# moritzmeister/hops-examples

Hardware: AMD Instinct MI355X
Metric: images/sec MNIST CNN + steps/sec Chicago-taxi DNN at 1/2/4/8 MI355X (higher is better)
Workload: dtype bf16; 1 GPU; model=MNIST CNN (experiment.mirrored model, 1394282 params), Adadelta(1.0), global_batch=32, per_gpu_batch=32, parallelism=dp1, engine=PersistentMnistStep, hipgraph=False, steps_per_execution=32, warmup_steps_run=5

## Files before the change

csrc/ops/bindings.cpp:

```cpp
#include <pybind11/pybind11.h>
#include <pybind11/stl.h>

#include <algorithm>
#include <stdexcept>
#include <string>
#include <tuple>
#include <utility>
#include <vector>

#if defined(HOPSX_DEBUG) && HOPSX_DEBUG
#define HOPSX_DEBUG_BUILD 1
#else
#define HOPSX_DEBUG_BUILD 0
#endif

#include "ops_api.h"
extern "C" int hopsx_mnist_persist_occupancy(int dp);
extern "C" void hopsx_mnist_persist_reload_knobs();
extern "C" int hopsx_pad_cin(const float* w, long R, int C, int cp, float* out, void* out16, hipStream_t st);
extern "C" int hopsx_unpad_cin_add(float* gpad, long R, int C, int cp, float* tgt, hipStream_t st);

namespace py = pybind11;
extern "C" void hopsx_mlp_head_debug(void* p);
extern "C" int hopsx_conv2d_bwd_pair_opt(const void* dy, const void* w, const int* geom, void* dx, const void* yprev,
// ... 168 lines not shown
    }
    persist_slots[slot] = PersistSlot{std::move(p), std::move(iv), std::move(fv)};
    return slot;
  });
  m.def("mnist_persist_slot", [](int slot, u st) {
    if (slot < 0 || slot >= (int)persist_slots.size()) return (int)hipErrorInvalidValue;
    const PersistSlot& a = persist_slots[slot];
    return hopsx_mnist_persist(a.p.data(), (int)a.p.size(), a.iv.data(), (int)a.iv.size(), a.fv.data(),
                               (int)a.fv.size(), S(st));
  });
  m.def("mnist_eval", [](std::vector<uint64_t> p, std::vector<long> iv, std::vector<float> fv, u st) {
    return hopsx_mnist_eval(p.data(), (int)p.size(), iv.data(), (int)iv.size(), fv.data(), (int)fv.size(), S(st));
  });
  m.def("mnist_eval_tile", []() { return hopsx_mnist_eval_tile(); });
  m.def("mnist_persist_reload_knobs", []() { hopsx_mnist_persist_reload_knobs(); });
  m.def("mnist_persist_occupancy", [](int dp) { return hopsx_mnist_persist_occupancy(dp); });
  m.def("pad_cin", [](u w, long R, int C, int cp, u out, u out16, u st) {
    return hopsx_pad_cin(P<float>(w), R, C, cp, P<float>(out), P<void>(out16), S(st));
  });
  m.def("unpad_cin_add", [](u g, long R, int C, int cp, u tgt, u st) {
    return hopsx_unpad_cin_add(P<float>(g), R, C, cp, P<float>(tgt), S(st));
  });
  m.def("mnist_persist_geom", []() {
    std::vector<long> g(23);
    hopsx_mnist_persist_geom(g.data());
    return g;
  });
  m.def("widedeep_step", [](std::vector<uint64_t> p, std::vector<long> iv, std::vector<float> fv, u st) {
    return hopsx_widedeep_step(p.data(), (int)p.size(), iv.data(), (int)iv.size(), fv.data(), (int)fv.size(),
                               S(st));
  });
  m.def("conv2d_fwd_pool_ok", [](std::vector<int> g, int act, int pk) { return hopsx_conv_fwd_pool_ok(g.data(), act, pk); });
  m.def("conv2d_fwd_pool", [](u x, u w, std::vector<int> g, u out, u am, u bias, int act, float p, u rng,
                              unsigned salt, int pk, u st) {
    return hopsx_conv2d_fwd_pool(P<void>(x), P<void>(w), g.data(), P<void>(out), P<void>(am), P<float>(bias), act, p,
                                 P<unsigned long long>(rng), salt, pk, S(st));
  });
  m.def("conv2d_fwd_pool_in_ok", [](std::vector<int> g0, std::vector<int> g, int act) {
    return hopsx_conv_fwd_pool_in_ok(g0.data(), g.data(), act);
  });
  m.def("conv2d_fwd_pool_in", [](u x0, float xscale, float xshift, u w0, u b0, int act0, std::vector<int> g0, u y1,
                                 u w, std::vector<int> g, u out, u am, u bias, int act, float p, u rng, unsigned salt,
                                 u st) {
    return hopsx_conv2d_fwd_pool_in(P<void>(x0), xscale, xshift, P<void>(w0), P<float>(b0), act0, g0.data(),
                                    P<void>(y1), P<void>(w), g.data(), P<void>(out), P<void>(am), P<float>(bias), act,
                                    p, P<unsigned long long>(rng), salt, S(st));
  });
// ... 227 lines not shown
```

csrc/ops/mnist_persist.hip:

```cpp
#include "common.h"
#include "optim_core.h"

namespace mnistp {

constexpr int B = 32;
constexpr int C1 = 32, C2 = 64, HID = 128, NCLS = 10;
constexpr int PH = 13, NPOS = PH * PH;
constexpr int KIN = NPOS * C2;
constexpr int NCONV = C2 * 128 + C2 + C1 * 4 + C1;
constexpr int OFF_B2 = C2 * 128, OFF_W1 = OFF_B2 + C2, OFF_B1 = OFF_W1 + C1 * 4;
constexpr int SLICE = 52, NSLICE = (NCONV + SLICE - 1) / SLICE;
constexpr int NRED = 19;
constexpr int NHEAD = B;
constexpr int GRID = NPOS + NHEAD;
constexpr int PAY = 272;
constexpr int PAY_DH = 0, PAY_H = 128, PAY_DL = 256, PAY_LOSS = 268, PAY_COR = 269;
constexpr int FL_A = 0, FL_B = 256, FL_C = 512, FL_D = 768, FL_WORDS = 1024;
constexpr int FL_EPOCH = FL_WORDS - 2;
constexpr int D_F32 = OFF_B2 * 2;
constexpr int D_BYTES = D_F32 + (NCONV - OFF_B2) * 4;
constexpr int TGB_N = NHEAD * (HID / 2);
constexpr int TG_WORDS = 2 * 2 * TGB_N;
static_assert(FL_WORDS % 2 == 0 && TGB_N % 256 == 0, "granules are 8-B aligned; every thread owns TGB_N / 256");

constexpr int W1S = 72, W2S = 136, C1S = 40, PLS = 72, DHS = 136, DCS = 136;

constexpr int L_W1 = 0;
constexpr int L_W2 = L_W1 + HID * W1S * 2;
constexpr int L_CW1 = L_W2 + C2 * W2S * 2;
constexpr int L_CB1 = L_CW1 + C1 * 4 * 4;
constexpr int L_CB2 = L_CB1 + C1 * 4;
constexpr int L_XIN = L_CB2 + C2 * 4;
constexpr int L_C1 = L_XIN + B * 16 * 4;
constexpr int L_POOL = L_C1 + B * 9 * C1S * 2;
constexpr int L_AM = L_POOL + B * PLS * 2;
constexpr int L_DH = L_AM + B * C2;
constexpr int L_DC2 = L_DH + B * DHS * 2;
constexpr int L_STG = L_DC2 + C2 * DCS * 2;
constexpr int L_RED = L_STG + NCONV * 4;
constexpr int L_SL = L_RED + 1024 * 4;
constexpr int L_KEEP = L_SL + 3 * 64 * 4;
constexpr int LDS_BYTES = L_KEEP + B * C2;

constexpr int H_W2 = 0;
constexpr int H_B2 = H_W2 + 3 * NCLS * HID * 4;
constexpr int H_B1 = H_B2 + 3 * 16 * 4;
// ... 230 lines not shown
__device__ __forceinline__ unsigned ecode(int phase, int s) {
  return 0x80000000u | ((unsigned)phase << 24) | (((unsigned)s & 0xFFFu) << 12) | (blockIdx.x & 0xFFFu);
}

__device__ __forceinline__ bf16_raw f2bf(float f) { return __builtin_bit_cast(bf16_raw, (__bf16)f); }

__device__ __forceinline__ bf16x8 lds8(const bf16_raw* p) { return *(const bf16x8*)p; }
__device__ __forceinline__ bf16x8 lds_tr(const bf16_raw* p1, const bf16_raw* p2) {
  const bf16x4 v1 = __builtin_amdgcn_ds_read_tr16_b64_v4i16((lds_v4_ptr)(p1));
  const bf16x4 v2 = __builtin_amdgcn_ds_read_tr16_b64_v4i16((lds_v4_ptr)(p2));
  return (bf16x8){v1[0], v1[1], v1[2], v1[3], v2[0], v2[1], v2[2], v2[3]};
}
__device__ __forceinline__ f32x4 mfma(bf16x8 a, bf16x8 b, f32x4 c) {
  return __builtin_amdgcn_mfma_f32_16x16x32_bf16(a, b, c, 0, 0, 0);
}

__device__ __forceinline__ long conv_idx(const Args& a, int j) {
  if (j < OFF_B2) return a.off[2] + j;
  if (j < OFF_W1) return a.off[3] + (j - OFF_B2);
  if (j < OFF_B1) return a.off[0] + (j - OFF_W1);
  return a.off[1] + (j - OFF_B1);
}

__device__ __forceinline__ void stamp(const Args& a, int s, int ph) {
  if (a.dbg && threadIdx.x == 0) a.dbg[((long)blockIdx.x * a.nsteps + s) * 16 + ph] = (unsigned long long)wall_clock64();
}

__device__ __forceinline__ void granule_store(unsigned long long* g, unsigned epoch, unsigned value) {
  __hip_atomic_store((gu64*)g, ((unsigned long long)epoch << 32) | value, __ATOMIC_RELAXED, __HIP_MEMORY_SCOPE_AGENT);
}
__device__ __forceinline__ unsigned long long granule_load(const unsigned long long* g) {
  return __hip_atomic_load((gu64*)g, __ATOMIC_RELAXED, __HIP_MEMORY_SCOPE_AGENT);
}
__device__ __forceinline__ bool gate_tags(const unsigned long long* g, int gi, unsigned epoch, int need, unsigned* err,
                                       unsigned code, int* s_ok, long long tmo) {
  if (threadIdx.x < 64) {
    const int lane = threadIdx.x;
    const bool mine = lane < NHEAD;
    int good = 1;
    const long long t0 = wall_clock64();
    for (unsigned spins = 0;; ++spins) {
      const unsigned e = flag_load(err);
      const unsigned long long x = mine ? granule_load(g + lane * (HID / 2) + gi) : 0ull;
      const bool hit = mine && (unsigned)(x >> 32) == epoch;
      if (__popcll(__ballot(hit)) >= need) break;
      if (__builtin_amdgcn_readfirstlane(e) != 0u) {
        good = 0;
        break;
      }
      if ((spins & 15u) == 15u && wall_clock64() - t0 > tmo) {
        if (lane == 0) atomicCAS(err, 0u, code);
        good = 0;
        break;
      }
      __builtin_amdgcn_s_sleep(1);
    }
    if (lane == 0) *s_ok = good;
  }
  __syncthreads();
  const int v = *s_ok;
  return v != 0;
}
template <int N, class F>
__device__ __forceinline__ bool sweep_tags(const unsigned long long* g, int tid, unsigned epoch, unsigned* err,
                                        unsigned code, int* s_fail, long long tmo, F put) {
  unsigned pend = (1u << N) - 1u;
  unsigned long long x[N];
#pragma unroll
  for (int k = 0; k < N; ++k) x[k] = granule_load(g + tid + 256 * k);
  unsigned e = flag_load(err);
  const long long t0 = wall_clock64();
  for (unsigned spins = 0;; ++spins) {
#pragma unroll
    for (int k = 0; k < N; ++k)
      if (((pend >> k) & 1u) && (unsigned)(x[k] >> 32) == epoch) {
        put(tid + 256 * k, (unsigned)x[k]);
        pend &= ~(1u << k);
      }
    if (!__any(pend != 0u)) break;
    bool bad = __builtin_amdgcn_readfirstlane(e) != 0u;
    if (!bad && (spins & 15u) == 15u && wall_clock64() - t0 > tmo) {
      if ((threadIdx.x & 63) == 0) atomicCAS(err, 0u, code);
      bad = true;
    }
    if (bad) {
      if ((threadIdx.x & 63) == 0) *s_fail = 1;
      break;
    }
#pragma unroll
    for (int k = 0; k < N; ++k)
      if ((pend >> k) & 1u) x[k] = granule_load(g + tid + 256 * k);
    e = flag_load(err);
// ... 41 lines not shown
        g2[ii][j][r] = a.s2[ai];
        W1[n * W1S + co] = f2bf(wm[ii][j][r]);
      }
  auto put_conv = [&](int j, float v) {
    if (j < OFF_B2) W2[(j >> 7) * W2S + (j & 127)] = f2bf(v);
    else if (j < OFF_W1) CB2[j - OFF_B2] = v;
    else if (j < OFF_B1) CW1[j - OFF_W1] = v;
    else CB1[j - OFF_B1] = v;
  };
  {
    constexpr int NJ = (NCONV + 255) / 256;
    float cv[NJ];
#pragma unroll
    for (int q = 0; q < NJ; ++q) {
      const int j = tid + 256 * q;
      cv[q] = j < NCONV ? a.master[conv_idx(a, j)] : 0.f;
    }
#pragma unroll
    for (int q = 0; q < NJ; ++q) {
      const int j = tid + 256 * q;
      if (j < NCONV) put_conv(j, cv[q]);
    }
  }
  const bool owner = p < NSLICE;
  if (owner && tid < SLICE) {
    const int e = p * SLICE + tid;
    if (e < NCONV) {
      const long ci = conv_idx(a, e);
      SLm[tid] = a.master[ci];
      SL1[tid] = a.s1[ci];
      SL2[tid] = a.s2[ci];
    }
  }
  const int xb = tid >> 3, xr = (tid >> 1) & 3, xh = tid & 1;
  auto xload = [&](int s) -> unsigned {
    const long bt = (long)((cur0 + s) % a.nbatch);
    const unsigned char* q = a.xs + (bt * B + xb) * 784 + (2 * ph + xr) * 28 + 2 * pw + 2 * xh;
    return *(const unsigned short*)q;
  };
  unsigned xv = xload(0);
  const float P = a.drop_p, inv = P > 0.f ? 1.f / (1.f - P) : 1.f;
  unsigned char* KEEP = smem + L_KEEP;
  auto draw_keep = [&](int s) {
    const unsigned long long ctr = ctr0 + (unsigned long long)s;
    const uint64_t dkey = (uint64_t)seed ^ ((uint64_t)a.salt * 0xD1B54A32D192ED03ull) ^
                          ((uint64_t)ctr * 0x8CB92BA72F3D8DD7ull);
    for (int e = threadIdx.x; e < B * C2; e += 256) {
      const int b = e >> 6, co = e & 63;
      const long gb = (long)a.rank * B + b;
      KEEP[e] = P > 0.f ? (unsigned char)(uniform01(dkey, (uint64_t)((gb * NPOS + p) * C2 + co)) >= P) : 1;
    }
  };
  draw_keep(0);
  __syncthreads();

  for (int s = 0; s < a.nsteps; ++s) {
    const unsigned ep = (unsigned)(eb + (unsigned long long)s + 1ull);
    const int par = s & 1;
    int oz;
    asm volatile("v_mov_b32 %0, 0" : "=v"(oz));
    const int tid = threadIdx.x + oz, lane = tid & 63, w = tid >> 6, fr = lane & 15, fq = lane >> 4;
    const int tq = fr >> 2, tp = fr & 3, xb = tid >> 3, xr = (tid >> 1) & 3, xh = tid & 1;
    stamp(a, s, 0);
    XIN[xb * 16 + xr * 4 + 2 * xh] = (float)(xv & 0xFFu) * a.xscale + a.xshift;
    XIN[xb * 16 + xr * 4 + 2 * xh + 1] = (float)(xv >> 8) * a.xscale + a.xshift;
    __syncthreads();
    {
      const int ci = tid & 31, bg = tid >> 5;
      const float k0 = CW1[ci * 4 + 0], k1 = CW1[ci * 4 + 1], k2 = CW1[ci * 4 + 2], k3 = CW1[ci * 4 + 3];
      const float bias = CB1[ci];
#pragma unroll
      for (int u = 0; u < 4; ++u) {
        const int b = bg * 4 + u;
        const float* xi = XIN + b * 16;
#pragma unroll
        for (int py = 0; py < 3; ++py)
#pragma unroll
          for (int px = 0; px < 3; ++px) {
            float v = bias;
            v = fmaf(xi[py * 4 + px], k0, v);
            v = fmaf(xi[py * 4 + px + 1], k1, v);
            v = fmaf(xi[(py + 1) * 4 + px], k2, v);
            v = fmaf(xi[(py + 1) * 4 + px + 1], k3, v);
            C1[(b * 9 + py * 3 + px) * C1S + ci] = f2bf(fmaxf(v, 0.f));
          }
      }
    }
    __syncthreads();
    {
      f32x4 acc[2][4];
#pragma unroll
      for (int ii = 0; ii < 2; ++ii)
#pragma unroll
        for (int j = 0; j < 4; ++j) acc[ii][j] = (f32x4){0.f, 0.f, 0.f, 0.f};
#pragma unroll
      for (int kk = 0; kk < 4; ++kk) {
        const int di = kk >> 1, dj = kk & 1;
        bf16x8 af[2];
#pragma unroll
        for (int ii = 0; ii < 2; ++ii) {
          const int b = 4 * (2 * w + ii) + (fr >> 2), q = fr & 3;
          const int pos = ((q >> 1) + di) * 3 + (q & 1) + dj;
          af[ii] = lds8(C1 + (b * 9 + pos) * C1S + fq * 8);
        }
#pragma unroll
        for (int j = 0; j < 4; ++j) {
          const bf16x8 bfr = lds8(W2 + (j * 16 + fr) * W2S + kk * 32 + fq * 8);
#pragma unroll
          for (int ii = 0; ii < 2; ++ii) acc[ii][j] = mfma(af[ii], bfr, acc[ii][j]);
        }
      }
// ... 53 lines not shown
    }
    __syncthreads();
    {
      const auto R = rsrc(a.slabA + ((long)par * NPOS + p) * (B * HID));
#pragma unroll
      for (int k = 0; k < 4; ++k) {
        const int idx = tid + 256 * k;
        st_sc1(R, idx * 16, *(const f32x4*)(STG + idx * 4));
      }
      drain();
      __syncthreads();
      if (tid == 0) flag_store(a.flags + FL_A + p, ep);
    }
    const unsigned gep = (unsigned)(xs0 + s + 1);
    if constexpr (DP) {
      const int c0 = w * 16 + 4 * tp;
      const f32x4 f = __builtin_bit_cast(f32x4, lds_tr(POOL + (8 * fq + tq) * PLS + c0, POOL + (8 * fq + tq + 4) * PLS + c0));
      for (int r = 0; r < a.world; ++r) {
        if (r == a.rank) continue;
        st_sys(rsrc(a.xbuf[r] + XO_POOL + (par * XMAX + xslot(a, r)) * XS_POOL + (long)p * 4096), (w * 64 + lane) * 16, f);
      }
    }
    if (s + 1 < a.nsteps) xv = xload(s + 1);
    stamp(a, s, 2);
    if (a.hand & 1) {
      const unsigned long long* TB = (const unsigned long long*)(a.flags + FL_WORDS) + par * TGB_N;
      const unsigned code = s ? ecode(2, s) : ecode(12, 0);
      const long long tmo = s ? a.tmo : a.tmo0;
      if (!gate_tags(TB, p & (HID / 2 - 1), ep, (a.hand >> 8), a.err, code, s_ok, tmo)) return;
      if (!sweep_tags<TGB_N / 256>(TB, tid, ep, a.err, code, s_ok + 2, tmo, [&](int idx, unsigned v) {
            *(unsigned*)(DH + (idx >> 6) * DHS + 2 * (idx & 63)) = v;
          }))
        return;
      if constexpr (DP) {
        drain();
        __syncthreads();
        if (tid < 64) raise_peers(a, XF_POOL + p, NPOS, gep);
      }
      stamp(a, s, 3);
    } else {
    if (!wait_all(a.flags + FL_B, NHEAD, ep, a.err, s ? ecode(2, s) : ecode(12, 0), a.acquire, s_ok,
                  s ? a.tmo : a.tmo0, a.pollw_b, a.stagger, (a.hand & 2)))
      return;
    if constexpr (DP) {
      drain();
      __syncthreads();
      if (tid < 64) raise_peers(a, XF_POOL + p, NPOS, gep);
    }
    stamp(a, s, 3);
    {
      const auto R = rsrc(a.slabB + (long)par * NHEAD * PAY);
#pragma unroll
      for (int k = 0; k < 4; ++k) {
        const int idx = tid + 256 * k, b = idx >> 5, n4 = idx & 31;
        const f32x4 v = ld_sc1(R, (b * PAY + PAY_DH + n4 * 4) * 4);
        *(bf16x4*)(DH + b * DHS + n4 * 4) =
            (bf16x4){(short)f2bf(v[0]), (short)f2bf(v[1]), (short)f2bf(v[2]), (short)f2bf(v[3])};
      }
    }
    __syncthreads();
    }
    f32x4 gw[2][4], dp[2];
    {
      if constexpr (!DP) {
#pragma unroll
      for (int ii = 0; ii < 2; ++ii) {
        const int n0 = (2 * w + ii) * 16 + 4 * tp;
        const bf16x8 af = lds_tr(DH + (8 * fq + tq) * DHS + n0, DH + (8 * fq + tq + 4) * DHS + n0);
#pragma unroll
        for (int j = 0; j < 4; ++j) {
          const int c0 = j * 16 + 4 * tp;
          const bf16x8 bfr = lds_tr(POOL + (8 * fq + tq) * PLS + c0, POOL + (8 * fq + tq + 4) * PLS + c0);
          gw[ii][j] = mfma(af, bfr, (f32x4){0.f, 0.f, 0.f, 0.f});
        }
      }
      }
      dp[0] = dp[1] = (f32x4){0.f, 0.f, 0.f, 0.f};
#pragma unroll
      for (int kk = 0; kk < 4; ++kk) {
        const int k1 = kk * 32 + 8 * fq + tq;
        const bf16x8 bfr = lds_tr(W1 + k1 * W1S + w * 16 + 4 * tp, W1 + (k1 + 4) * W1S + w * 16 + 4 * tp);
#pragma unroll
        for (int i = 0; i < 2; ++i) dp[i] = mfma(lds8(DH + (i * 16 + fr) * DHS + kk * 32 + fq * 8), bfr, dp[i]);
      }
    }
// ... 87 lines not shown
#pragma unroll
        for (int py = 0; py < 3; ++py)
#pragma unroll
          for (int px = 0; px < 3; ++px) {
            const int pos = py * 3 + px;
            const float dd = (short)C1[(b * 9 + pos) * C1S + ci] > 0 ? d[pos] : 0.f;
            gk[0] = fmaf(dd, xi[py * 4 + px], gk[0]);
            gk[1] = fmaf(dd, xi[py * 4 + px + 1], gk[1]);
            gk[2] = fmaf(dd, xi[(py + 1) * 4 + px], gk[2]);
            gk[3] = fmaf(dd, xi[(py + 1) * 4 + px + 1], gk[3]);
            gk[4] += dd;
          }
      }
#pragma unroll
      for (int k = 0; k < 5; ++k) {
        gk[k] += __shfl_xor(gk[k], 16, 64);
        gk[k] += __shfl_xor(gk[k], 32, 64);
      }
      if (fq == 0) {
#pragma unroll
        for (int k = 0; k < 5; ++k) RED[(mh * 32 + ci) * 5 + k] = gk[k];
      }
    }
    __syncthreads();
    if (tid < 32 * 5) {
      const int ci = tid / 5, k = tid - ci * 5;
      const float v = RED[ci * 5 + k] + RED[(32 + ci) * 5 + k];
      if (k < 4) STG[OFF_W1 + ci * 4 + k] = v;
      else STG[OFF_B1 + ci] = v;
    }
    __syncthreads();
    stamp(a, s, 5);
    {
      const auto R = rsrc(a.slabC + ((long)par * NPOS + p) * NCONV);
      const int idx = OFF_B2 / 4 + tid;
      if (idx < NCONV / 4) st_sc1(R, idx * 16, *(const f32x4*)(STG + idx * 4));
      drain();
      __syncthreads();
      if (tid == 0) flag_store(a.flags + FL_C + p, ep);
    }
    stamp(a, s, 6);
    if (owner) {
      if (!wait_all(a.flags + FL_C, NPOS, ep, a.err, ecode(3, s), a.acquire, s_ok, a.tmo, a.pollw_c, a.stagger, (a.hand & 2)))
        return;
      stamp(a, s, 7);
      const int e0 = p * SLICE;
      if (tid < 13 * NRED) {
        const int j = tid % 13, g = tid / 13;
        f32x4 acc = (f32x4){0.f, 0.f, 0.f, 0.f};
        if (e0 + 4 * j < NCONV) {
          const auto R = rsrc(a.slabC + (long)par * NPOS * NCONV);
          constexpr int NK = (NPOS + NRED - 1) / NRED;
          f32x4 v[NK];
#pragma unroll
          for (int k = 0; k < NK; ++k) {
            const int pp = g + NRED * k;
            v[k] = pp < NPOS ? ld_sc1(R, (pp * NCONV + e0 + 4 * j) * 4) : (f32x4){0.f, 0.f, 0.f, 0.f};
          }
#pragma unroll
          for (int k = 0; k < NK; ++k) acc += v[k];
        }
        *(f32x4*)(RED + g * SLICE + 4 * j) = acc;
      }
      __syncthreads();
      const int e = e0 + tid;
// ... 75 lines not shown
#pragma unroll
          for (int ii = 0; ii < 2; ++ii)
            af[b][ii] = __builtin_bit_cast(bf16x8, ld_sys(XD, (int)(r * XS_DHT) + ((2 * w + ii) * 64 + lane) * 16));
#pragma unroll
          for (int j = 0; j < 4; ++j)
            bfr[b][j] = __builtin_bit_cast(bf16x8, ld_sys(XP, (int)(r * XS_POOL) + (j * 64 + lane) * 16));
        }
      };
#pragma unroll
      for (int r = 0; r < PF - 1; ++r)
        if (r < a.world) fetch(r, r);
#pragma unroll
      for (int r = 0; r < XMAX; ++r) {
        if (r < a.world) {
          if (r + PF - 1 < XMAX && r + PF - 1 < a.world) fetch(r + PF - 1, (r + PF - 1) % PF);
#pragma unroll
          for (int ii = 0; ii < 2; ++ii)
#pragma unroll
            for (int j = 0; j < 4; ++j)
              gw[ii][j] += mfma(af[r % PF][ii], bfr[r % PF][j], (f32x4){0.f, 0.f, 0.f, 0.f});
        }
      }
    }
#pragma unroll
    for (int ii = 0; ii < 2; ++ii)
#pragma unroll
      for (int j = 0; j < 4; ++j)
#pragma unroll
        for (int r = 0; r < 4; ++r) {
          wm[ii][j][r] = adadelta(wm[ii][j][r], gw[ii][j][r] * hp.gscale, g1[ii][j][r], g2[ii][j][r], hp);
          W1[((2 * w + ii) * 16 + fq * 4 + r) * W1S + j * 16 + fr] = f2bf(wm[ii][j][r]);
        }
    if (s + 1 < a.nsteps) draw_keep(s + 1);
    stamp(a, s, 9);
    if (!wait_all(a.flags + FL_D, NSLICE, ep, a.err, ecode(4, s), a.acquire, s_ok, a.tmo, a.pollw_d, a.stagger,
                  (a.hand & 2)))
      return;
    stamp(a, s, 10);
    {
      const auto R = rsrc((const unsigned char*)a.slabD + (long)par * D_BYTES);
      constexpr int NB = OFF_B2 * 2 / 16;
      constexpr int NF = (NCONV - OFF_B2) / 4;
      f32x4 dv[NB / 256 + 1];
#pragma unroll
      for (int k = 0; k < NB / 256; ++k) dv[k] = ld_sc1(R, (tid + 256 * k) * 16);
      dv[NB / 256] = tid < NF ? ld_sc1(R, D_F32 + tid * 16) : (f32x4){0.f, 0.f, 0.f, 0.f};
#pragma unroll
      for (int k = 0; k < NB / 256; ++k) {
        const int c = tid + 256 * k;
        *(f32x4*)(W2 + (c >> 4) * W2S + (c & 15) * 8) = dv[k];
      }
      if (tid < NF) {
        const int j = OFF_B2 + tid * 4;
        float* dst = j < OFF_W1 ? CB2 + (j - OFF_B2) : (j < OFF_B1 ? CW1 + (j - OFF_W1) : CB1 + (j - OFF_B1));
        *(f32x4*)dst = dv[NB / 256];
      }
    }
    __syncthreads();
    stamp(a, s, 11);
  }

#pragma unroll
  for (int ii = 0; ii < 2; ++ii)
#pragma unroll
    for (int j = 0; j < 4; ++j)
#pragma unroll
      for (int r = 0; r < 4; ++r) {
        const int n = (2 * w + ii) * 16 + fq * 4 + r, co = j * 16 + fr;
        const long ai = a.off[4] + (long)n * KIN + p * C2 + co;
        a.master[ai] = wm[ii][j][r];
        a.s1[ai] = g1[ii][j][r];
        a.s2[ai] = g2[ii][j][r];
        a.shadow[ai] = f2bf(wm[ii][j][r]);
      }
  if (owner && tid < SLICE) {
    const int e = p * SLICE + tid;
    if (e < NCONV) {
      const long ci = conv_idx(a, e);
      a.master[ci] = SLm[tid];
      a.s1[ci] = SL1[tid];
      a.s2[ci] = SL2[tid];
      a.shadow[ci] = f2bf(SLm[tid]);
    }
  }
  stamp(a, a.nsteps - 1, 14);
  if (p == 0 && tid == 0) {
    if constexpr (DP) a.xstep[0] = xs0 + a.nsteps;
    a.cursor[0] = (cur0 + a.nsteps) % a.nbatch;
    *(unsigned long long*)(a.flags + FL_EPOCH) = eb + (unsigned long long)a.nsteps;
    a.rng[1] = ctr0 + (unsigned long long)a.nsteps;
    if (a.step_dev) a.step_dev[0] += (float)a.nsteps;
  }
}

template <bool DP>
__device__ __forceinline__ void head_wg(const Args& a, unsigned char* smem, int* s_ok, const OptHP& hp,
                                        long long cur0, long long xs0, unsigned long long eb) {
  const int i = blockIdx.x - NPOS;
  const int tid = threadIdx.x, lane = tid & 63;
  float* HW = (float*)(smem + H_W2);
  float* HW1 = HW + NCLS * HID;
  float* HW2 = HW1 + NCLS * HID;
  float* HB2 = (float*)(smem + H_B2);
  float* HB1 = (float*)(smem + H_B1);
  float* RED = (float*)(smem + H_RED);
  float* HH = (float*)(smem + H_H);
// ... 348 lines not shown
  a.rng = (unsigned long long*)p[7];
  a.step_dev = (float*)p[8];
  a.hp_dev = (const float*)p[9];
  a.slabA = (float*)p[10];
  a.slabB = (float*)p[11];
  a.slabC = (float*)p[12];
  a.slabD = (float*)p[13];
  a.flags = (unsigned*)p[14];
  a.err = (unsigned*)p[15];
  a.out = (float*)p[16];
  a.dbg = (unsigned long long*)p[17];
  for (int k = 0; k < 8; ++k) a.off[k] = iv[k];
  a.nbatch = iv[8];
  a.salt = (unsigned)iv[9];
  a.nsteps = (int)iv[10];
  a.acquire = (int)iv[12];
  a.world = world;
  a.rank = rank;
  a.loopback = (int)iv[15];
  a.xfence = (int)iv[17];
  a.tmo = (long long)iv[16] * 100000ll;
  a.tmo0 = a.tmo;
  static int kn_ok = 0, kn_pollw, kn_stagger, kn_a, kn_b, kn_c, kn_d, kn_head1w, kn_memset, kn_coop;
  static int kn_tagged, kn_gate, kn_poll1;
  static long kn_start_ms;
  if (!kn_ok || g_persist_reload) {
    auto pw = [&](const char* name, long dflt) {
      const long v = hopsx_env_int(name, dflt);
      return (int)(v >= 1 && v <= 4 ? v : 1);
    };
    kn_pollw = pw("HOPSX_PERSIST_POLLW", 1);
    kn_stagger = (int)hopsx_env_int("HOPSX_PERSIST_STAGGER", 12);
    kn_a = pw("HOPSX_PERSIST_POLLW_A", kn_pollw);
    kn_b = pw("HOPSX_PERSIST_POLLW_B", kn_pollw);
    kn_c = pw("HOPSX_PERSIST_POLLW_C", 4);
    kn_d = pw("HOPSX_PERSIST_POLLW_D", kn_pollw);
    kn_head1w = (int)hopsx_env_int("HOPSX_PERSIST_HEAD1W", 1);
    kn_memset = (int)hopsx_env_int("HOPSX_PERSIST_MEMSET", 0);
    kn_coop = (int)hopsx_env_int("HOPSX_PERSIST_COOP", 0);
    kn_start_ms = hopsx_env_int("HOPSX_PERSIST_START_MS", 50);
    kn_tagged = hopsx_env_int("HOPSX_PERSIST_TAGGED", 1) != 0;
    const long gt = hopsx_env_int("HOPSX_PERSIST_GATE", NHEAD / 2);
    kn_gate = (int)(gt >= 1 && gt <= NHEAD ? gt : NHEAD / 2);
    kn_poll1 = hopsx_env_int("HOPSX_PERSIST_POLL1", 1) != 0;
    kn_ok = 1;
    g_persist_reload = 0;
  }
  a.pollw = kn_pollw;
  a.stagger = kn_stagger;
  a.pollw_a = kn_a;
  a.pollw_b = kn_b;
  a.pollw_c = kn_c;
  a.pollw_d = kn_d;
  a.head1w = kn_head1w;
  a.hand = kn_tagged | (kn_poll1 << 1) | (kn_gate << 8);
  if (kn_start_ms > 0 && kn_start_ms * 100000ll < a.tmo) a.tmo0 = kn_start_ms * 100000ll;
  a.inv_gb = 1.f / (float)(world * B);
  if (dp) {
    a.xstep = (long long*)p[18];
    for (int r = 0; r < world; ++r) {
      a.xbuf[r] = (unsigned char*)p[19 + r];
      a.xflag[r] = (unsigned*)p[19 + world + r];
      if (!a.xbuf[r] || !a.xflag[r] || ((uint64_t)a.xbuf[r] & 15)) return (int)hipErrorInvalidValue;
    }
  }
  a.drop_p = fv[0];
  a.xscale = fv[1];
  a.xshift = fv[2];
  a.hp = OptHP{fv[3], fv[4], fv[5], fv[6], fv[7], 0.f, 0.f, 0.f};
  static bool attr[2] = {false, false};
  const void* fn = dp ? (const void*)mnist_persist_k<true> : (const void*)mnist_persist_k<false>;
  if (!attr[dp]) {
    const hipError_t e = hipFuncSetAttribute(fn, hipFuncAttributeMaxDynamicSharedMemorySize, LDS_BYTES);
    if (e != hipSuccess) return (int)e;
    attr[dp] = true;
  }
  if (kn_memset) {
    const hipError_t e = hipMemsetAsync(a.flags, 0, FL_WORDS * sizeof(unsigned), st);
// ... 29 lines not shown
  g[0] = B;
  g[1] = NPOS;
  g[2] = NHEAD;
  g[3] = GRID;
  g[4] = NCONV;
  g[5] = NSLICE;
  g[6] = SLICE;
  g[7] = PAY;
  g[8] = FL_WORDS;
  g[9] = LDS_BYTES;
  g[10] = D_BYTES;
  g[11] = X_BYTES;
  g[12] = XF_WORDS;
  g[13] = XMAX;
  g[14] = XO_POOL;
  g[15] = XS_POOL;
  g[16] = XO_DHT;
  g[17] = XS_DHT;
  g[18] = XO_FC2;
  g[19] = XS_FC2;
  g[20] = XO_CONV;
  g[21] = XS_CONV;
  g[22] = TG_WORDS;
}
```

hops_examples_amd/runtime/persist.py:

```python
from __future__ import annotations

import os

import torch

_GEOM = None


def _ext():
    from ..ops import _C

    return _C.ext()


def geometry() -> dict:
    global _GEOM
    if _GEOM is None:
        g = _ext().mnist_persist_geom()
        _GEOM = dict(zip(["batch", "npos", "nhead", "grid", "nconv", "nslice", "slice", "pay", "flag_words",
                          "lds_bytes", "d_bytes", "x_bytes", "xflag_words", "max_ranks", "xo_pool", "xs_pool",
                          "xo_dht", "xs_dht", "xo_fc2", "xs_fc2", "xo_conv", "xs_conv", "tag_words"], g))
    return _GEOM


class PersistentError(RuntimeError):
    pass


def flagship_layers(model):
    from .. import nn as hnn
    from ..models.mnist import MirroredMnistCNN

    names = ("conv1", "conv2", "pool", "fc1", "fc2")
    L = [getattr(model, n, None) for n in names]
    if any(x is None for x in L):
        return None
    c1, c2, pool, f1, f2 = L

    def conv_ok(c, cin, cout):
        return (isinstance(c, hnn.Conv2d) and c.in_channels == cin and c.out_channels == cout
                and tuple(c.kernel_size) == (2, 2) and c.activation == "relu" and c.bias is not None
                and c.cfg.get("stride", 1) in (1, (1, 1)) and c.cfg.get("padding", 0) in (0, "valid", (0, 0))
                and c.cfg.get("dilation", 1) in (1, (1, 1)))

    def dense_ok(d, fin, fout, act):
# ... 7 lines not shown
    return L if ok and type(model).forward is MirroredMnistCNN.forward else None


def _device_cus(dev) -> int:
    return int(torch.cuda.get_device_properties(dev).multi_processor_count)


def _occupancy(dp: bool) -> int:
    return int(_ext().mnist_persist_occupancy(int(dp)))


def launchable(dev, world: int = 1) -> tuple[bool, str]:
    g = geometry()
    cus = _device_cus(dev)
    if cus < g["grid"]:
        return False, f"{cus} CUs < the persistent grid of {g['grid']} workgroups"
    occ = _occupancy(world > 1)
    if occ < 1:
        return False, f"occupancy {occ} workgroups per CU"
    return True, "ok"


class PersistentMnistStep:
    PARAMS = ("conv1.weight", "conv1.bias", "conv2.weight", "conv2.bias", "fc1.weight", "fc1.bias",
              "fc2.weight", "fc2.bias")

    @staticmethod
    def supported(model, opt, batch: int, world: int = 1) -> bool:
        from ..optim import Adadelta

        if os.environ.get("HOPSX_PERSIST", "1") != "1":
            return False
        if world > 1 and (os.environ.get("HOPSX_PERSIST_DP", "1") != "1" or world > geometry()["max_ranks"]):
            return False
        a = getattr(opt, "arena", None)
        if not (isinstance(opt, Adadelta) and batch == 32 and a is not None and a.device.type == "cuda"
                and a.shadow is not None and opt._sl.start == 0 and opt._sl.stop >= a.numel and model.training
                and flagship_layers(model) is not None):
            return False
        return launchable(a.device, world)[0]

    def __init__(self, model, opt, steps_per_launch: int = 32, debug_stamps: bool = False, world: int | None = None,
                 loopback: int = 0, timeout_s: float | None = None, exchange=None):
        from ..ops.functional import rng_state
        from ..parallel import dist as hdist

        a = opt.arena
        self.model, self.opt, self.arena = model, opt, a
        dev = a.device
        self.device = dev
        g = geometry()
        self.geom = g
        named = dict(model.named_parameters())
        self.offs = [int(named[n]._hx_off) for n in self.PARAMS]
        self.s1 = a.state("adadelta_s0")
        self.s2 = a.state("adadelta_s1")
        self.spl = max(1, int(os.environ.get("HOPSX_PERSIST_STEPS", steps_per_launch)))
        f32 = dict(device=dev, dtype=torch.float32)
        B, npos, nh = g["batch"], g["npos"], g["nhead"]
        self.slabA = torch.empty(2 * npos * B * 128, **f32)
        self.slabB = torch.empty(2 * nh * g["pay"], **f32)
        self.slabC = torch.empty(2 * npos * g["nconv"], **f32)
        self.slabD = torch.empty(2 * g["d_bytes"] // 4, **f32)
        self._flagbuf = torch.zeros(g["flag_words"] + g["tag_words"], device=dev, dtype=torch.int32)
        self.flags = self._flagbuf[:g["flag_words"]]
        self.tags = self._flagbuf[g["flag_words"]:]
        self.err = torch.zeros(4, device=dev, dtype=torch.int32)
        self.out = torch.zeros(2 * self.spl, **f32)
        self.cursor = torch.zeros(1, device=dev, dtype=torch.int64)
        self.rng = rng_state(dev)
        self.dbg = torch.zeros(g["grid"] * self.spl * 16, device=dev, dtype=torch.int64) if debug_stamps else None
        self.acquire = int(os.environ.get("HOPSX_PERSIST_ACQUIRE", "0"))
        self.loopback = int(loopback)
        self.xfence = int(os.environ.get("HOPSX_PERSIST_XFENCE", "0"))
        if exchange is not None:
            self.world, self.rank = int(exchange.world), 0
        elif self.loopback > 1:
            self.world, self.rank = self.loopback, 0
        else:
            self.world = int(world) if world is not None else hdist.world_size()
            self.rank = hdist.rank() if self.world > 1 else 0
        if self.world > g["max_ranks"]:
            raise ValueError(f"the persistent step supports <= {g['max_ranks']} ranks")
        default_t = "60" if self.world > 1 else "2"
        self.timeout_ms = int(1000 * float(timeout_s or os.environ.get("HOPSX_PERSIST_TIMEOUT_S", default_t)))
        self._xptrs: list[int] = []
        self._owned: list[int] = []
        self._opened: list[int] = []
        self.exchange = exchange
        self.selftest_report: dict | None = None
        if exchange is not None:
            self.xstep = torch.zeros(1, device=self.device, dtype=torch.int64)
            exchange.attach(self)
        elif self.world > 1:
# ... 304 lines not shown
    def eager(self, x, y):
        return self(x, y)

    def prepare_resident(self, xs, ys, n=None) -> None:
        nb = self._check_data(xs, ys)
        if n:
            self.opt.sync_hp()
            hp = [float(v) for v in self.opt._hp()]
            for k in {min(int(n), self.spl), int(n) % self.spl} - {0}:
                self._arg_slot(self._launch_key(xs, ys, nb, k, hp), xs, ys, nb, k, hp)

    def losses(self, k: int) -> torch.Tensor:
        return self.out[: 2 * k].view(k, 2)

    def check(self) -> None:
        e = int(self.err[0].item()) & 0xFFFFFFFF
        if e:
            self._flagbuf.zero_()
            phase, step, wg = (e >> 24) & 0x7F, (e >> 12) & 0xFFF, e & 0xFFF
            if phase == 12:
                raise PersistentError(f"mnist_persist: the grid's workgroups were not co-resident (workgroup {wg} "
                                      "waited out step 0's local hand-off: another kernel holds CUs this launch "
                                      "needs); arena state of the failed launch is partial")
            raise PersistentError(f"mnist_persist: hand-off wait timed out (phase {phase}, step {step}, "
                                  f"workgroup {wg}); arena state of the failed launch is partial")

    def phase_stamps(self, k: int) -> torch.Tensor:
        if self.dbg is None:
            raise RuntimeError("construct with debug_stamps=True")
        return self.dbg.view(self.geom["grid"], self.spl, 16)[:, :k]


_M32 = 0xFFFFFFFF


def _mix32(x: torch.Tensor) -> torch.Tensor:
    x = x ^ (x >> 16)
    x = (x * 0x7FEB352D) & _M32
    x = x ^ (x >> 15)
    x = (x * 0x846CA68B) & _M32
    return x ^ (x >> 16)


def dropout_keep(seed: int, ctr: int, salt: int, idx: torch.Tensor, p: float) -> torch.Tensor:
    m64 = (1 << 64) - 1
    key = (seed ^ ((salt * 0xD1B54A32D192ED03) & m64) ^ ((ctr * 0x8CB92BA72F3D8DD7) & m64)) & m64
    ka, kb = key & _M32, key >> 32
    h = _mix32((_mix32((idx & _M32) ^ ka) + kb) & _M32)
    return (h & 0xFFFFFF).to(torch.float64) * (1.0 / 16777216.0) >= p


class _RoundFwd(torch.autograd.Function):

# ... 94 lines not shown
```

Before: 1.361 million images/sec.

## Split conv gradient hand-off so small conv params reduce via tags and overlap conv1

Adds a split mode, on by default, to the persistent MNIST step. The small conv parameters (conv2 bias, conv1 weight and bias) get their gradients reduced through per-position tagged granules and a few dedicated owners. Only the conv2 weight goes through the sliced slab C/D path, and the next step's input and conv1 forward is computed while waiting for the conv2 weight broadcast. The dropout mask draw and the fc1 Adadelta update are also moved earlier to overlap with the hand-off waits. In exchange, the flag buffer and the control flow grow, and there are new tag regions and extra wait phases that could add polling cost.

```diff
diff --git a/csrc/ops/bindings.cpp b/csrc/ops/bindings.cpp
--- a/csrc/ops/bindings.cpp
+++ b/csrc/ops/bindings.cpp
@@ -214,7 +214,7 @@
     return hopsx_unpad_cin_add(P<float>(g), R, C, cp, P<float>(tgt), S(st));
   });
   m.def("mnist_persist_geom", []() {
-    std::vector<long> g(23);
+    std::vector<long> g(30);
     hopsx_mnist_persist_geom(g.data());
     return g;
   });
diff --git a/csrc/ops/mnist_persist.hip b/csrc/ops/mnist_persist.hip
--- a/csrc/ops/mnist_persist.hip
+++ b/csrc/ops/mnist_persist.hip
@@ -22,6 +22,18 @@
 constexpr int TGB_N = NHEAD * (HID / 2);
 constexpr int TG_WORDS = 2 * 2 * TGB_N;
 static_assert(FL_WORDS % 2 == 0 && TGB_N % 256 == 0, "granules are 8-B aligned; every thread owns TGB_N / 256");
+constexpr int NSMALL = NCONV - OFF_B2;
+constexpr int NSL2 = (OFF_B2 + SLICE - 1) / SLICE;
+constexpr int NSOWN = NSMALL / 2;
+constexpr int FL_C1 = FL_WORDS + TG_WORDS, FC1_WORDS = 256;
+constexpr int TGC_N = NSMALL * NPOS;
+constexpr int TGC_OFF = FL_C1 + FC1_WORDS, TGC_WORDS = 2 * 2 * TGC_N;
+constexpr int TGD_OFF = TGC_OFF + TGC_WORDS, TGD_WORDS = 2 * 2 * NSMALL;
+constexpr int SP_WORDS = FC1_WORDS + TGC_WORDS + TGD_WORDS;
+constexpr int NSTAMP = 20;
+static_assert(NSMALL % 2 == 0 && NSOWN <= NSL2 && NSL2 <= NSLICE && 2 * NPOS <= 512 && NSMALL <= 256 &&
+                  TGC_OFF % 2 == 0 && TGD_OFF % 2 == 0 && SLICE + 2 <= 64 && SLICE % 2 == 0,
+              "split geometry: 8-B aligned granules, two sweep passes per small owner, state rows of 64");
 
 constexpr int W1S = 72, W2S = 136, C1S = 40, PLS = 72, DHS = 136, DCS = 136;
 
@@ -298,8 +310,8 @@
   return a.off[1] + (j - OFF_B1);
 }
 
-__device__ __forceinline__ void stamp(const Args& a, int s, int ph) {
-  if (a.dbg && threadIdx.x == 0) a.dbg[((long)blockIdx.x * a.nsteps + s) * 16 + ph] = (unsigned long long)wall_clock64();
+__device__ __forceinline__ void stamp(const Args& a, int s, int ph, int t = 0) {
+  if (a.dbg && threadIdx.x == t) a.dbg[((long)blockIdx.x * a.nsteps + s) * NSTAMP + ph] = (unsigned long long)wall_clock64();
 }
 
 __device__ __forceinline__ void granule_store(unsigned long long* g, unsigned epoch, unsigned value) {
@@ -339,11 +351,14 @@
 }
 template <int N, class F>
 __device__ __forceinline__ bool sweep_tags(const unsigned long long* g, int tid, unsigned epoch, unsigned* err,
-                                        unsigned code, int* s_fail, long long tmo, F put) {
-  unsigned pend = (1u << N) - 1u;
+                                        unsigned code, int* s_fail, long long tmo, F put, int n = 256 * N) {
+  unsigned pend = 0u;
   unsigned long long x[N];
 #pragma unroll
-  for (int k = 0; k < N; ++k) x[k] = granule_load(g + tid + 256 * k);
+  for (int k = 0; k < N; ++k) {
+    if (tid + 256 * k < n) pend |= 1u << k;
+    x[k] = tid + 256 * k < n ? granule_load(g + tid + 256 * k) : 0ull;
+  }
   unsigned e = flag_load(err);
   const long long t0 = wall_clock64();
   for (unsigned spins = 0;; ++spins) {
@@ -431,15 +446,21 @@
       if (j < NCONV) put_conv(j, cv[q]);
     }
   }
-  const bool owner = p < NSLICE;
-  if (owner && tid < SLICE) {
+  const bool split = DP ? false : (a.hand & 4) != 0;
+  if (p < (split ? NSL2 : NSLICE) && tid < SLICE) {
     const int e = p * SLICE + tid;
-    if (e < NCONV) {
+    if (e < (split ? OFF_B2 : NCONV)) {
       const long ci = conv_idx(a, e);
       SLm[tid] = a.master[ci];
       SL1[tid] = a.s1[ci];
       SL2[tid] = a.s2[ci];
     }
+  }
+  if (split && p < NSOWN && tid < 2) {
+    const long ci = conv_idx(a, OFF_B2 + 2 * p + tid);
+    SLm[SLICE + tid] = a.master[ci];
+    SL1[SLICE + tid] = a.s1[ci];
+    SL2[SLICE + tid] = a.s2[ci];
   }
   const int xb = tid >> 3, xr = (tid >> 1) & 3, xh = tid & 1;
   auto xload = [&](int s) -> unsigned {
@@ -471,6 +492,7 @@
     const int tid = threadIdx.x + oz, lane = tid & 63, w = tid >> 6, fr = lane & 15, fq = lane >> 4;
     const int tq = fr >> 2, tp = fr & 3, xb = tid >> 3, xr = (tid >> 1) & 3, xh = tid & 1;
     stamp(a, s, 0);
+    auto input_conv1 = [&]() {
     XIN[xb * 16 + xr * 4 + 2 * xh] = (float)(xv & 0xFFu) * a.xscale + a.xshift;
     XIN[xb * 16 + xr * 4 + 2 * xh + 1] = (float)(xv >> 8) * a.xscale + a.xshift;
     __syncthreads();
@@ -495,7 +517,11 @@
           }
       }
     }
-    __syncthreads();
+    };
+    if (!split || s == 0) {
+      input_conv1();
+      __syncthreads();
+    }
     {
       f32x4 acc[2][4];
 #pragma unroll
@@ -595,6 +621,7 @@
       }
     }
     if (s + 1 < a.nsteps) xv = xload(s + 1);
+    if (s + 1 < a.nsteps) draw_keep(s + 1);
     stamp(a, s, 2);
     if (a.hand & 1) {
       const unsigned long long* TB = (const unsigned long long*)(a.flags + FL_WORDS) + par * TGB_N;
@@ -634,6 +661,17 @@
     __syncthreads();
     }
     f32x4 gw[2][4], dp[2];
+    auto fc1_update = [&]() {
+#pragma unroll
+      for (int ii = 0; ii < 2; ++ii)
+#pragma unroll
+        for (int j = 0; j < 4; ++j)
+#pragma unroll
+          for (int r = 0; r < 4; ++r) {
+            wm[ii][j][r] = adadelta(wm[ii][j][r], gw[ii][j][r] * hp.gscale, g1[ii][j][r], g2[ii][j][r], hp);
+            W1[((2 * w + ii) * 16 + fq * 4 + r) * W1S + j * 16 + fr] = f2bf(wm[ii][j][r]);
+          }
+    };
     {
       if constexpr (!DP) {
 #pragma unroll
@@ -767,7 +805,23 @@
         for (int k = 0; k < 5; ++k) RED[(mh * 32 + ci) * 5 + k] = gk[k];
       }
     }
+    if (split) drain();
     __syncthreads();
+    if (split) {
+      if (tid == 0) flag_store(a.flags + FL_C1 + p, ep);
+      stamp(a, s, 12);
+      unsigned long long* TC = (unsigned long long*)(a.flags + TGC_OFF) + (long)par * TGC_N;
+      if (tid < 32 * 5) {
+        const int ci = tid / 5, k = tid - ci * 5;
+        const float v = RED[ci * 5 + k] + RED[(32 + ci) * 5 + k];
+        const int j = k < 4 ? OFF_W1 - OFF_B2 + ci * 4 + k : OFF_B1 - OFF_B2 + ci;
+        granule_store(TC + j * NPOS + p, ep, __float_as_uint(v));
+      } else if (tid < 32 * 5 + C2) {
+        const int j = tid - 32 * 5;
+        granule_store(TC + j * NPOS + p, ep, __float_as_uint(STG[OFF_B2 + j]));
+      }
+      stamp(a, s, 5);
+    } else {
     if (tid < 32 * 5) {
       const int ci = tid / 5, k = tid - ci * 5;
       const float v = RED[ci * 5 + k] + RED[(32 + ci) * 5 + k];
@@ -784,8 +838,83 @@
       __syncthreads();
       if (tid == 0) flag_store(a.flags + FL_C + p, ep);
     }
+    }
     stamp(a, s, 6);
-    if (owner) {
+    if constexpr (!DP) fc1_update();
+    if (split) {
+      constexpr int NK = (NPOS + NRED - 1) / NRED;
+      const int e0 = p * SLICE, j13 = tid % 13, g13 = tid / 13;
+      const bool ldr = tid < 13 * NRED && e0 + 4 * j13 < OFF_B2;
+      if (split && p < NSOWN) {
+        const unsigned long long* TC =
+            (const unsigned long long*)(a.flags + TGC_OFF) + (long)par * TGC_N + 2 * p * NPOS;
+        if (!sweep_tags<2>(TC, tid, ep, a.err, ecode(11, s), s_ok + 2, a.tmo,
+                           [&](int idx, unsigned x) { STG[idx] = __uint_as_float(x); }, 2 * NPOS))
+          return;
+        if (w == 1) {
+          const int q = lane / NRED, g = lane - q * NRED;
+          float acc = 0.f;
+#pragma unroll
+          for (int k = 0; k < NK; ++k) {
+            const int pp = g + NRED * k;
+            if (pp < NPOS) acc += STG[q * NPOS + pp];
+          }
+          float gs = 0.f;
+#pragma unroll
+          for (int gg = 0; gg < NRED; ++gg) gs += __shfl(acc, (lane & 1) * NRED + gg, 64);
+          if (lane < 2) {
+            const float wn = adadelta(SLm[SLICE + lane], gs * hp.gscale, SL1[SLICE + lane], SL2[SLICE + lane], hp);
+            SLm[SLICE + lane] = wn;
+            granule_store((unsigned long long*)(a.flags + TGD_OFF) + par * NSMALL + 2 * p + lane, ep,
+                          __float_as_uint(wn));
+          }
+          stamp(a, s, 15, 64);
+        }
+      }
+      if (p < (split ? NSL2 : NSLICE)) {
+        if (!wait_all(a.flags + FL_C1, NPOS, ep, a.err, ecode(10, s), a.acquire, s_ok, a.tmo, a.pollw_c, a.stagger,
+                      (a.hand & 2)))
+          return;
+        stamp(a, s, 7);
+        if (tid < 13 * NRED) {
+          f32x4 acc = (f32x4){0.f, 0.f, 0.f, 0.f};
+          if (ldr) {
+            const auto R = rsrc(a.slabC + (long)par * NPOS * NCONV);
+            f32x4 v[NK];
+#pragma unroll
+            for (int k = 0; k < NK; ++k) {
+              const int pp = g13 + NRED * k;
+              v[k] = pp < NPOS ? ld_sc1(R, (pp * NCONV + e0 + 4 * j13) * 4) : (f32x4){0.f, 0.f, 0.f, 0.f};
+            }
+#pragma unroll
+            for (int k = 0; k < NK; ++k) acc += v[k];
+          }
+          *(f32x4*)(RED + g13 * SLICE + 4 * j13) = acc;
+        }
+        __syncthreads();
+        const int e = e0 + tid;
+        if (tid < SLICE) {
+          float gs = 0.f;
+          for (int g = 0; g < NRED; ++g) gs += RED[g * SLICE + tid];
+          float wn = 0.f;
+          if (e < OFF_B2) {
+            SLm[tid] = adadelta(SLm[tid], gs * hp.gscale, SL1[tid], SL2[tid], hp);
+            wn = SLm[tid];
+          }
+          const float wnext = __shfl_down(wn, 1, 64);
+          unsigned char* D = (unsigned char*)a.slabD + (long)par * D_BYTES;
+          if (e < OFF_B2 && !(tid & 1))
+            __hip_atomic_store((gu32*)(D + e * 2), (unsigned)f2bf(wn) | ((unsigned)f2bf(wnext) << 16),
+                               __ATOMIC_RELAXED, __HIP_MEMORY_SCOPE_AGENT);
+        }
+        if (w == 0) {
+          drain();
+          if (lane == 0) flag_store(a.flags + FL_D + p, ep);
+        }
+        stamp(a, s, 8);
+      }
+    } else
+    if (p < (split ? NSL2 : NSLICE)) {
       if (!wait_all(a.flags + FL_C, NPOS, ep, a.err, ecode(3, s), a.acquire, s_ok, a.tmo, a.pollw_c, a.stagger, (a.hand & 2)))
         return;
       stamp(a, s, 7);
@@ -907,17 +1036,36 @@
         }
       }
     }
-#pragma unroll
-    for (int ii = 0; ii < 2; ++ii)
-#pragma unroll
-      for (int j = 0; j < 4; ++j)
-#pragma unroll
-        for (int r = 0; r < 4; ++r) {
-          wm[ii][j][r] = adadelta(wm[ii][j][r], gw[ii][j][r] * hp.gscale, g1[ii][j][r], g2[ii][j][r], hp);
-          W1[((2 * w + ii) * 16 + fq * 4 + r) * W1S + j * 16 + fr] = f2bf(wm[ii][j][r]);
-        }
-    if (s + 1 < a.nsteps) draw_keep(s + 1);
+    if constexpr (DP) fc1_update();
     stamp(a, s, 9);
+    if (split) {
+      const unsigned long long* TD = (const unsigned long long*)(a.flags + TGD_OFF) + par * NSMALL;
+      if (!sweep_tags<1>(TD, tid, ep, a.err, ecode(13, s), s_ok + 2, a.tmo,
+                         [&](int idx, unsigned x) {
+                           const int j = OFF_B2 + idx;
+                           float* dst = j < OFF_W1 ? CB2 + (j - OFF_B2) : (j < OFF_B1 ? CW1 + (j - OFF_W1) : CB1 + (j - OFF_B1));
+                           *dst = __uint_as_float(x);
+                         },
+                         NSMALL))
+        return;
+      stamp(a, s, 16);
+      if (s + 1 < a.nsteps) input_conv1();
+      stamp(a, s, 17);
+      if (!wait_all(a.flags + FL_D, NSL2, ep, a.err, ecode(4, s), a.acquire, s_ok, a.tmo, a.pollw_d, a.stagger,
+                    (a.hand & 2)))
+        return;
+      stamp(a, s, 10);
+      const auto R = rsrc((const unsigned char*)a.slabD + (long)par * D_BYTES);
+      constexpr int NB = OFF_B2 * 2 / 16;
+      f32x4 dv[NB / 256];
+#pragma unroll
+      for (int k = 0; k < NB / 256; ++k) dv[k] = ld_sc1(R, (tid + 256 * k) * 16);
+#pragma unroll
+      for (int k = 0; k < NB / 256; ++k) {
+        const int c = tid + 256 * k;
+        *(f32x4*)(W2 + (c >> 4) * W2S + (c & 15) * 8) = dv[k];
+      }
+    } else {
     if (!wait_all(a.flags + FL_D, NSLICE, ep, a.err, ecode(4, s), a.acquire, s_ok, a.tmo, a.pollw_d, a.stagger,
                   (a.hand & 2)))
       return;
@@ -941,6 +1089,7 @@
         *(f32x4*)dst = dv[NB / 256];
       }
     }
+    }
     __syncthreads();
     stamp(a, s, 11);
   }
@@ -958,15 +1107,22 @@
         a.s2[ai] = g2[ii][j][r];
         a.shadow[ai] = f2bf(wm[ii][j][r]);
       }
-  if (owner && tid < SLICE) {
+  if (p < (split ? NSL2 : NSLICE) && tid < SLICE) {
     const int e = p * SLICE + tid;
-    if (e < NCONV) {
+    if (e < (split ? OFF_B2 : NCONV)) {
       const long ci = conv_idx(a, e);
       a.master[ci] = SLm[tid];
       a.s1[ci] = SL1[tid];
       a.s2[ci] = SL2[tid];
       a.shadow[ci] = f2bf(SLm[tid]);
     }
+  }
+  if (split && p < NSOWN && tid < 2) {
+    const long ci = conv_idx(a, OFF_B2 + 2 * p + tid);
+    a.master[ci] = SLm[SLICE + tid];
+    a.s1[ci] = SL1[SLICE + tid];
+    a.s2[ci] = SL2[SLICE + tid];
+    a.shadow[ci] = f2bf(SLm[SLICE + tid]);
   }
   stamp(a, a.nsteps - 1, 14);
   if (p == 0 && tid == 0) {
@@ -1361,7 +1517,7 @@
   a.tmo = (long long)iv[16] * 100000ll;
   a.tmo0 = a.tmo;
   static int kn_ok = 0, kn_pollw, kn_stagger, kn_a, kn_b, kn_c, kn_d, kn_head1w, kn_memset, kn_coop;
-  static int kn_tagged, kn_gate, kn_poll1;
+  static int kn_tagged, kn_gate, kn_poll1, kn_split;
   static long kn_start_ms;
   if (!kn_ok || g_persist_reload) {
     auto pw = [&](const char* name, long dflt) {
@@ -1382,6 +1538,7 @@
     const long gt = hopsx_env_int("HOPSX_PERSIST_GATE", NHEAD / 2);
     kn_gate = (int)(gt >= 1 && gt <= NHEAD ? gt : NHEAD / 2);
     kn_poll1 = hopsx_env_int("HOPSX_PERSIST_POLL1", 1) != 0;
+    kn_split = hopsx_env_int("HOPSX_PERSIST_SPLIT", 1) != 0;
     kn_ok = 1;
     g_persist_reload = 0;
   }
@@ -1392,7 +1549,7 @@
   a.pollw_c = kn_c;
   a.pollw_d = kn_d;
   a.head1w = kn_head1w;
-  a.hand = kn_tagged | (kn_poll1 << 1) | (kn_gate << 8);
+  a.hand = kn_tagged | (kn_poll1 << 1) | (kn_split << 2) | (kn_gate << 8);
   if (kn_start_ms > 0 && kn_start_ms * 100000ll < a.tmo) a.tmo0 = kn_start_ms * 100000ll;
   a.inv_gb = 1.f / (float)(world * B);
   if (dp) {
@@ -1468,4 +1625,11 @@
   g[20] = XO_CONV;
   g[21] = XS_CONV;
   g[22] = TG_WORDS;
-}
+  g[23] = SP_WORDS;
+  g[24] = FC1_WORDS;
+  g[25] = TGC_WORDS;
+  g[26] = TGD_WORDS;
+  g[27] = NSL2;
+  g[28] = NSOWN;
+  g[29] = NSTAMP;
+}
diff --git a/hops_examples_amd/runtime/persist.py b/hops_examples_amd/runtime/persist.py
--- a/hops_examples_amd/runtime/persist.py
+++ b/hops_examples_amd/runtime/persist.py
@@ -19,8 +19,20 @@
         g = _ext().mnist_persist_geom()
         _GEOM = dict(zip(["batch", "npos", "nhead", "grid", "nconv", "nslice", "slice", "pay", "flag_words",
                           "lds_bytes", "d_bytes", "x_bytes", "xflag_words", "max_ranks", "xo_pool", "xs_pool",
-                          "xo_dht", "xs_dht", "xo_fc2", "xs_fc2", "xo_conv", "xs_conv", "tag_words"], g))
+                          "xo_dht", "xs_dht", "xo_fc2", "xs_fc2", "xo_conv", "xs_conv", "tag_words", "split_words",
+                          "c1_flag_words", "small_c_words", "small_d_words", "nslice_split", "nsmall_owners",
+                          "stamps"], g))
     return _GEOM
+
+
+def flag_regions(g: dict) -> dict:
+    out, o = {}, 0
+    for name, key in (("flags", "flag_words"), ("tags", "tag_words"), ("c1_flags", "c1_flag_words"),
+                      ("small_c", "small_c_words"), ("small_d", "small_d_words")):
+        out[name] = (o, int(g[key]))
+        o += int(g[key])
+    out["total"] = (0, o)
+    return out
 
 
 class PersistentError(RuntimeError):
@@ -74,6 +86,12 @@
 
 
 class PersistentMnistStep:
+    PHASES = {1: "A, fc1 partials at the heads", 2: "B, dh at the positions", 3: "C, conv gradients at the slice owners",
+              4: "D, conv parameters at the positions", 5: "B at the heads", 6: "cross-rank conv slice sums",
+              7: "cross-rank dh", 8: "cross-rank pooled activations", 9: "cross-rank head gradients",
+              10: "C1, conv2 weight gradient at its slice owners (split form)",
+              11: "small conv gradients at their owners (split form, tagged)", 12: "co-residency",
+              13: "small conv parameters at the positions (split form, tagged)"}
     PARAMS = ("conv1.weight", "conv1.bias", "conv2.weight", "conv2.bias", "fc1.weight", "fc1.bias",
               "fc2.weight", "fc2.bias")
 
@@ -114,14 +132,16 @@
         self.slabB = torch.empty(2 * nh * g["pay"], **f32)
         self.slabC = torch.empty(2 * npos * g["nconv"], **f32)
         self.slabD = torch.empty(2 * g["d_bytes"] // 4, **f32)
-        self._flagbuf = torch.zeros(g["flag_words"] + g["tag_words"], device=dev, dtype=torch.int32)
-        self.flags = self._flagbuf[:g["flag_words"]]
-        self.tags = self._flagbuf[g["flag_words"]:]
+        reg = flag_regions(g)
+        self._flagbuf = torch.zeros(reg["total"][1], device=dev, dtype=torch.int32)
+        view = lambda n: self._flagbuf[reg[n][0]:reg[n][0] + reg[n][1]]
+        self.flags, self.tags = view("flags"), view("tags")
+        self.c1_flags, self.small_c, self.small_d = view("c1_flags"), view("small_c"), view("small_d")
         self.err = torch.zeros(4, device=dev, dtype=torch.int32)
         self.out = torch.zeros(2 * self.spl, **f32)
         self.cursor = torch.zeros(1, device=dev, dtype=torch.int64)
         self.rng = rng_state(dev)
-        self.dbg = torch.zeros(g["grid"] * self.spl * 16, device=dev, dtype=torch.int64) if debug_stamps else None
+        self.dbg = torch.zeros(g["grid"] * self.spl * g["stamps"], device=dev, dtype=torch.int64) if debug_stamps else None
         self.acquire = int(os.environ.get("HOPSX_PERSIST_ACQUIRE", "0"))
         self.loopback = int(loopback)
         self.xfence = int(os.environ.get("HOPSX_PERSIST_XFENCE", "0"))
@@ -472,13 +492,14 @@
                 raise PersistentError(f"mnist_persist: the grid's workgroups were not co-resident (workgroup {wg} "
                                       "waited out step 0's local hand-off: another kernel holds CUs this launch "
                                       "needs); arena state of the failed launch is partial")
-            raise PersistentError(f"mnist_persist: hand-off wait timed out (phase {phase}, step {step}, "
+            what = self.PHASES.get(phase, "?")
+            raise PersistentError(f"mnist_persist: hand-off wait timed out (phase {phase}: {what}, step {step}, "
                                   f"workgroup {wg}); arena state of the failed launch is partial")
 
     def phase_stamps(self, k: int) -> torch.Tensor:
         if self.dbg is None:
             raise RuntimeError("construct with debug_stamps=True")
-        return self.dbg.view(self.geom["grid"], self.spl, 16)[:, :k]
+        return self.dbg.view(self.geom["grid"], self.spl, self.geom["stamps"])[:, :k]
 
 
 _M32 = 0xFFFFFFFF
```

After: 1.368 million images/sec (median of 6 runs). About the same (+0.5%).
